# m96-chan/PyGPUkit

Hardware: AMD Instinct MI355X
Metric: decode tokens/sec/GPU + prefill TFLOPS (% MFMA peak), Qwen3-0.6B bf16 (higher is better)
Workload: dtype bf16

## Files before the change

pygpukit_amd/csrc/flash_common.hip.h:

```cpp
#pragma once

#include <type_traits>

#include "attn_plan.h"
#include "pgk_device.hip.h"

namespace pgk {

typedef __bf16 bf16x8_fl __attribute__((ext_vector_type(8)));
typedef _Float16 f16x8_fl __attribute__((ext_vector_type(8)));
typedef float f32x16_fl __attribute__((ext_vector_type(16)));

template <class T> __device__ __forceinline__ f32x16_fl mfma32(const uint4& a, const uint4& b, f32x16_fl c);
template <> __device__ __forceinline__ f32x16_fl mfma32<bf16>(const uint4& a, const uint4& b, f32x16_fl c) {
    return __builtin_amdgcn_mfma_f32_32x32x16_bf16(__builtin_bit_cast(bf16x8_fl, a), __builtin_bit_cast(bf16x8_fl, b), c, 0, 0, 0);
}
template <> __device__ __forceinline__ f32x16_fl mfma32<f16>(const uint4& a, const uint4& b, f32x16_fl c) {
    return __builtin_amdgcn_mfma_f32_32x32x16_f16(__builtin_bit_cast(f16x8_fl, a), __builtin_bit_cast(f16x8_fl, b), c, 0, 0, 0);
}
template <class T> __device__ __forceinline__ uint32_t pack16x2(float lo, float hi);
template <> __device__ __forceinline__ uint32_t pack16x2<bf16>(float lo, float hi) { return pack_bf16x2(lo, hi); }
template <> __device__ __forceinline__ uint32_t pack16x2<f16>(float lo, float hi) {
    return (uint32_t)__builtin_bit_cast(uint16_t, static_cast<_Float16>(lo)) | ((uint32_t)__builtin_bit_cast(uint16_t, static_cast<_Float16>(hi)) << 16);
}

struct FlashPlain {};
struct FlashFull {};
struct FlashIrope {
    const void* positions;
    float attn_scale, floor_scale;
    int causal_offset;
    int pos_is_i64;
};
struct FlashAlibi {
    const float* slopes;
};

__device__ __forceinline__ int fl_v_off(int d, int c8) { return d * 128 + ((c8 ^ ((d >> 1) & 15)) << 3); }

struct FlashSplit {
    int nsplit;
    float* ml;
    void* o;
    uint8_t* q8;
    float* q8s;
};

template <class T, int D>
__global__ __launch_bounds__(256) void flash_merge_kernel(const float* ml, const T* po, T* out, int hq, int q_len, int nsplit, long long oh, long long os,
                                                          uint8_t* q8 = nullptr, float* q8s = nullptr) {
    constexpr int CPR = D / 8;
    const size_t gid = (size_t)blockIdx.x * 256 + threadIdx.x;
    const size_t nrow = (size_t)q_len * hq;
    if (gid >= nrow * CPR) return;
    const size_t rowi = gid / CPR;
    const int c = (int)(gid % CPR), qrow = (int)(rowi / hq), head = (int)(rowi % hq);
    float mstar = -INFINITY;
    for (int s2 = 0; s2 < nsplit; ++s2) mstar = fmaxf(mstar, ml[(((size_t)s2 * hq + head) * q_len + qrow) * 2]);
    float acc[8] = {0.f, 0.f, 0.f, 0.f, 0.f, 0.f, 0.f, 0.f}, den = 0.f;
    for (int s2 = 0; s2 < nsplit; ++s2) {
        const float* r = ml + (((size_t)s2 * hq + head) * q_len + qrow) * 2;
        const float w = (r[1] > 0.f) ? r[1] * __builtin_amdgcn_exp2f(r[0] - mstar) : 0.f;
        if (w > 0.f) {
            Vec<T> v;
            v.load(po + (((size_t)s2 * q_len + qrow) * hq + head) * D + c * 8);
            float f[8];
            v.to_float(f);
#pragma unroll
            for (int j = 0; j < 8; ++j) acc[j] = fmaf(w, f[j], acc[j]);
            den += w;
        }
    }
    const float inv = den > 0.f ? 1.f / den : 0.f;
#pragma unroll
    for (int j = 0; j < 8; ++j) acc[j] *= inv;
    Vec<T> v;
    v.from_float(acc);
    if constexpr (std::is_same<T, bf16>::value && D == 128) {
        if (q8 != nullptr) {
            v.to_float(acc);
            float amax = 0.f;
#pragma unroll
            for (int j = 0; j < 8; ++j) amax = fmaxf(amax, fabsf(acc[j]));
            amax = group16_max(amax);
            const float sc = amax > 0.f ? amax / 448.0f : 1.0f;
            uint2 o8;
            o8.x = pack_fp8x4(acc[0] / sc, acc[1] / sc, acc[2] / sc, acc[3] / sc);
            o8.y = pack_fp8x4(acc[4] / sc, acc[5] / sc, acc[6] / sc, acc[7] / sc);
            *reinterpret_cast<uint2*>(q8 + rowi * D + c * 8) = o8;
            if (c == 0) q8s[rowi] = sc;
            return;
        }
    }
    v.store(out + (size_t)head * oh + (size_t)qrow * os + c * 8);
}

template <class T, int D>
__global__ __launch_bounds__(256) void transpose_v_kernel(const T* v, T* vt, int kv_len, int kv_pad, long long kh, long long ks) {
    __shared__ uint16_t tile[64][D + 2];
    const int kv0 = blockIdx.x * 64, head = blockIdx.y;
    const T* vh = v + (size_t)head * kh;
    constexpr int NC = D / 8;
    for (int c = threadIdx.x; c < 64 * NC; c += 256) {
        const int r = c / NC, kc = c % NC;
        uint4 x = make_uint4(0, 0, 0, 0);
        if (kv0 + r < kv_len) x = *reinterpret_cast<const uint4*>(vh + (size_t)(kv0 + r) * ks + kc * 8);
        const uint32_t w[4] = {x.x, x.y, x.z, x.w};
#pragma unroll
        for (int j = 0; j < 4; ++j) {
            tile[r][kc * 8 + 2 * j] = (uint16_t)(w[j] & 0xFFFFu);
            tile[r][kc * 8 + 2 * j + 1] = (uint16_t)(w[j] >> 16);
        }
    }
    __syncthreads();
    T* oh = vt + (size_t)head * D * kv_pad;
    for (int c = threadIdx.x; c < D * 8; c += 256) {
        const int d = c >> 3, kc = c & 7;
        uint32_t w[4];
#pragma unroll
        for (int j = 0; j < 4; ++j) w[j] = (uint32_t)tile[kc * 8 + 2 * j][d] | ((uint32_t)tile[kc * 8 + 2 * j + 1][d] << 16);
        *reinterpret_cast<uint4*>(oh + (size_t)d * kv_pad + kv0 + kc * 8) = make_uint4(w[0], w[1], w[2], w[3]);
    }
}

}
```

pygpukit_amd/csrc/ops_flash.hip:

```cpp

#include "flash_common.hip.h"

namespace pgk {

template <int D> __device__ __forceinline__ int fl_k_off(int r, int c) { return r * (2 * D) + ((c ^ (r & (D / 8 - 1))) << 4); }

template <class T, int D, class X = FlashPlain>
__global__ __launch_bounds__(FL_THREADS, 2) void flash_fwd_kernel(const T* q, const T* k, const T* vt, T* out, int hq, int hkv,
                                                              int q_len, int kv_len, int kv_pad, float scale_log2e, FlashStrides sd,
                                                              FlashSplit sp, X ex) {
    constexpr bool IROPE = std::is_same<X, FlashIrope>::value;
    constexpr bool ALIBI = std::is_same<X, FlashAlibi>::value;
    constexpr bool FULL = std::is_same<X, FlashFull>::value;
    constexpr int NC = D / 8;
    constexpr int KS = D / 16;
    constexpr int DT = D / 32;
    constexpr int KCH = 64 * NC / FL_THREADS;
    constexpr int VCH = D * 8 / FL_THREADS;
    constexpr int K_BYTES = 64 * D * 2, V_BYTES = D * 128;
    extern __shared__ __attribute__((aligned(16))) char fl_smem[];
    auto Ks = [&](int buf) -> char* { return fl_smem + buf * K_BYTES; };
    auto Vs = [&](int buf) -> char* { return fl_smem + 2 * K_BYTES + buf * V_BYTES; };

    const int tid = threadIdx.x, lane = tid & 63, wid = tid >> 6, ql = lane & 31, h = lane >> 5;
    const int rep = hq / hkv, nqt = (q_len + FL_BQ - 1) / FL_BQ;
    const int id = blockIdx.x;
    const int kvh = id % hkv, rest = id / hkv;
    const int head = kvh * rep + rest % rep;
    const int rest2 = rest / rep;
    int order = rest2;
    const int nord = nqt * sp.nsplit;
    if (sp.nsplit > 1 && order >= nord / 2) order = nord / 2 + (nord - 1 - order);
    const int split = order % sp.nsplit;
    const int qt = nqt - 1 - order / sp.nsplit;
    const int qw0 = qt * FL_BQ + wid * 32;
    int mask_off = kv_len - q_len;
    if constexpr (IROPE) mask_off = ex.causal_offset;
    if constexpr (FULL) mask_off = kv_len;
    const int causal_off = mask_off;
    const T* qh = q + (size_t)head * sd.qh;
    const T* kh = k + (size_t)kvh * sd.kh;
    const T* vh = vt + (size_t)kvh * D * kv_pad;

    uint4 qf[KS];
    {
        const T* qrow = qh + (size_t)min(qw0 + ql, q_len - 1) * sd.qs + 8 * h;
        float qmul = scale_log2e;
        if constexpr (IROPE)
            qmul *= irope_temperature(irope_position(ex.positions, min(qw0 + ql, q_len - 1), ex.pos_is_i64), ex.attn_scale, ex.floor_scale);
#pragma unroll
        for (int ks = 0; ks < KS; ++ks) {
            Vec<T> v;
            v.load(qrow + ks * 16);
            float f[8];
            v.to_float(f);
#pragma unroll
            for (int j = 0; j < 8; ++j) f[j] *= qmul;
            v.from_float(f);
            qf[ks] = v.raw;
        }
    }
    f32x16_fl o[DT];
#pragma unroll
    for (int i = 0; i < DT; ++i)
#pragma unroll
        for (int r = 0; r < 16; ++r) o[i][r] = 0.f;
    float m_run = -INFINITY, l_run = 0.f;
    float slope2 = 0.f;
    if constexpr (ALIBI) slope2 = ex.slopes[head] * 1.4426950408889634f;

    const int q_last = min(qt * FL_BQ + FL_BQ - 1, q_len - 1);
    const int kv_end = min(kv_len, causal_off + q_last + 1);
    const int nt_all = (kv_end + FL_BKV - 1) / FL_BKV;
    const int t0 = (int)((long long)nt_all * split / sp.nsplit), t1 = (int)((long long)nt_all * (split + 1) / sp.nsplit);

    static_assert(KCH == VCH && (KCH == 2 || KCH == 4), "staging is written for D = 64 / 128");
    uint4 rk0, rk1, rk2, rk3, rv0, rv1, rv2, rv3;
    const int kr = tid / NC, kc16 = tid % NC;
    constexpr int KR_STEP = FL_THREADS / NC;
    const int vd = tid >> 3, vc = tid & 7;
    auto k_src = [&](int kv0, int i) { return kh + (size_t)min(kv0 + kr + KR_STEP * i, kv_len - 1) * sd.ks + kc16 * 8; };
    const uint32_t ko0 = (uint32_t)(kr * sd.ks + kc16 * 8), ko_step = (uint32_t)(KR_STEP * sd.ks);
    const uint32_t vo0 = (uint32_t)(vd * kv_pad + vc * 8), vo_step = (uint32_t)(32 * kv_pad);
    auto load_k = [&](int t) {
        const int kv0 = t * FL_BKV;
        if (kv0 + FL_BKV <= kv_len) {
            const T* kt = kh + (size_t)kv0 * sd.ks;
            rk0 = *reinterpret_cast<const uint4*>(kt + ko0);
            rk1 = *reinterpret_cast<const uint4*>(kt + ko0 + ko_step);
            if constexpr (KCH == 4) {
                rk2 = *reinterpret_cast<const uint4*>(kt + ko0 + 2 * ko_step);
                rk3 = *reinterpret_cast<const uint4*>(kt + ko0 + 3 * ko_step);
            }
        } else {
            rk0 = *reinterpret_cast<const uint4*>(k_src(kv0, 0));
            rk1 = *reinterpret_cast<const uint4*>(k_src(kv0, 1));
            if constexpr (KCH == 4) {
                rk2 = *reinterpret_cast<const uint4*>(k_src(kv0, 2));
                rk3 = *reinterpret_cast<const uint4*>(k_src(kv0, 3));
            }
        }
    };
    auto load_v = [&](int t) {
        const T* vtile = vh + t * FL_BKV;
        rv0 = *reinterpret_cast<const uint4*>(vtile + vo0);
        rv1 = *reinterpret_cast<const uint4*>(vtile + vo0 + vo_step);
        if constexpr (VCH == 4) {
            rv2 = *reinterpret_cast<const uint4*>(vtile + vo0 + 2 * vo_step);
            rv3 = *reinterpret_cast<const uint4*>(vtile + vo0 + 3 * vo_step);
        }
    };
    auto put_v = [&](char* base, int d, const uint4& x) {
        *reinterpret_cast<uint2*>(base + fl_v_off(d, 2 * vc)) = make_uint2(x.x, x.y);
        *reinterpret_cast<uint2*>(base + fl_v_off(d, 2 * vc + 1)) = make_uint2(x.z, x.w);
    };
    auto store_k = [&](int buf) {
        char* kb = Ks(buf);
        *reinterpret_cast<uint4*>(kb + fl_k_off<D>(kr, kc16)) = rk0;
        *reinterpret_cast<uint4*>(kb + fl_k_off<D>(kr + KR_STEP, kc16)) = rk1;
        if constexpr (KCH == 4) {
            *reinterpret_cast<uint4*>(kb + fl_k_off<D>(kr + 2 * KR_STEP, kc16)) = rk2;
            *reinterpret_cast<uint4*>(kb + fl_k_off<D>(kr + 3 * KR_STEP, kc16)) = rk3;
        }
    };
    auto store_v = [&](int buf) {
        char* vb = Vs(buf);
        put_v(vb, vd, rv0);
        put_v(vb, vd + 32, rv1);
        if constexpr (VCH == 4) {
            put_v(vb, vd + 64, rv2);
            put_v(vb, vd + 96, rv3);
        }
    };
    auto qk = [&](int buf, int kv0, f32x16_fl& s0, f32x16_fl& s1) {
        if constexpr (ALIBI) {
            const float base = slope2 * (float)(kv0 + 4 * h - (causal_off + qw0 + ql));
#pragma unroll
            for (int r = 0; r < 16; ++r) {
                s0[r] = fmaf(slope2, (float)((r & 3) + 8 * (r >> 2)), base);
                s1[r] = fmaf(slope2, (float)(32 + (r & 3) + 8 * (r >> 2)), base);
            }
        } else {
#pragma unroll
            for (int r = 0; r < 16; ++r) { s0[r] = 0.f; s1[r] = 0.f; }
        }
#pragma unroll
        for (int ks = 0; ks < KS; ++ks) {
            const uint4 a0 = *reinterpret_cast<const uint4*>(Ks(buf) + fl_k_off<D>(ql, 2 * ks + h));
            const uint4 a1 = *reinterpret_cast<const uint4*>(Ks(buf) + fl_k_off<D>(32 + ql, 2 * ks + h));
            s0 = mfma32<T>(a0, qf[ks], s0);
            s1 = mfma32<T>(a1, qf[ks], s1);
        }
    };
    auto live = [&](int t) -> bool { return t < t1 && t * FL_BKV <= causal_off + qw0 + 31; };

    f32x16_fl sc0, sc1;
    if (t0 < t1) {
        load_k(t0);
        load_v(t0);
        store_k(t0 & 1);
        store_v(t0 & 1);
    }
#pragma unroll
    for (int ks = 0; ks < KS; ++ks) asm volatile("" ::"v"(qf[ks].x), "v"(qf[ks].y), "v"(qf[ks].z), "v"(qf[ks].w));
    __syncthreads();
    typedef uint32_t fl_u32x2 __attribute__((ext_vector_type(2)));
    typedef __attribute__((address_space(3))) const volatile fl_u32x2* fl_lds_cv64;
    for (int t = t0; t < t1; ++t) {
        const int buf = t & 1, kv0 = t * FL_BKV;
        if (t + 1 < t1) { load_k(t + 1); load_v(t + 1); }
        const bool cur = live(t);
        if (cur) qk(buf, kv0, sc0, sc1);
        if (cur) {
            const bool need_mask = kv0 + FL_BKV - 1 > causal_off + qw0 || kv0 + FL_BKV > kv_len;
            const int lim = min(causal_off + qw0 + ql, kv_len - 1) - kv0 - 4 * h;
            float mx = -INFINITY;
            if (need_mask) {
#pragma unroll
                for (int r = 0; r < 16; ++r) {
                    const int kvl = (r & 3) + 8 * (r >> 2);
                    sc0[r] = kvl <= lim ? sc0[r] : -INFINITY;
                    sc1[r] = 32 + kvl <= lim ? sc1[r] : -INFINITY;
                }
            }
#pragma unroll
            for (int r = 0; r < 16; r += 2) mx = fmaxf(fmaxf(fmaxf(sc0[r], sc1[r]), fmaxf(sc0[r + 1], sc1[r + 1])), mx);
            mx = fmaxf(mx, __shfl_xor(mx, 32, 64));
            const float m_new = (mx > m_run + 6.0f || m_run == -INFINITY) ? fmaxf(m_run, mx) : m_run;
            const float m_use = m_new == -INFINITY ? 0.f : m_new;
            const bool moved = __builtin_amdgcn_ballot_w64(m_new != m_run) != 0;
            const float alpha = moved ? __builtin_amdgcn_exp2f(m_run - m_use) : 1.0f;
            float ls = 0.f;
#pragma unroll
            for (int r = 0; r < 16; ++r) {
                sc0[r] = __builtin_amdgcn_exp2f(sc0[r] - m_use);
                sc1[r] = __builtin_amdgcn_exp2f(sc1[r] - m_use);
                ls += sc0[r] + sc1[r];
            }
            l_run = l_run * alpha + ls;
            m_run = m_new;
            if (moved) {
#pragma unroll
                for (int i = 0; i < DT; ++i)
#pragma unroll
                    for (int r = 0; r < 16; ++r) o[i][r] *= alpha;
            }
            const char* vrow = Vs(buf) + ql * 128;
            const int vsw = (ql >> 1) & 15;
#pragma unroll
            for (int s = 0; s < 4; ++s) {
                uint4 pb;
                if (s < 2) {
                    pb = make_uint4(pack16x2<T>(sc0[8 * s + 0], sc0[8 * s + 1]), pack16x2<T>(sc0[8 * s + 2], sc0[8 * s + 3]),
                                    pack16x2<T>(sc0[8 * s + 4], sc0[8 * s + 5]), pack16x2<T>(sc0[8 * s + 6], sc0[8 * s + 7]));
                } else {
                    pb = make_uint4(pack16x2<T>(sc1[8 * (s - 2) + 0], sc1[8 * (s - 2) + 1]), pack16x2<T>(sc1[8 * (s - 2) + 2], sc1[8 * (s - 2) + 3]),
                                    pack16x2<T>(sc1[8 * (s - 2) + 4], sc1[8 * (s - 2) + 5]), pack16x2<T>(sc1[8 * (s - 2) + 6], sc1[8 * (s - 2) + 7]));
                }
#pragma unroll
                for (int i = 0; i < DT; ++i) {
                    const fl_u32x2 lo = *(fl_lds_cv64)(vrow + (((4 * s + h) ^ vsw) << 3) + i * 4096);
                    const fl_u32x2 hi = *(fl_lds_cv64)(vrow + (((4 * s + 2 + h) ^ vsw) << 3) + i * 4096);
                    o[i] = mfma32<T>(make_uint4(lo.x, lo.y, hi.x, hi.y), pb, o[i]);
                }
            }
        }
        if (t + 1 < t1) { store_k(buf ^ 1); store_v(buf ^ 1); }
        __syncthreads();
    }

    const float l_tot = l_run + __shfl_xor(l_run, 32, 64);
    const float inv = l_tot > 0.f ? 1.f / l_tot : 0.f;
    const int qrow = qw0 + ql;
    if constexpr (std::is_same<T, bf16>::value && D == 128 && std::is_same<X, FlashPlain>::value) {
        if (sp.q8 != nullptr && sp.nsplit == 1) {
            float amax = 0.f;
#pragma unroll
            for (int i = 0; i < DT; ++i)
#pragma unroll
                for (int e = 0; e < 16; ++e) {
                    o[i][e] = __uint_as_float(pack_bf16x2(o[i][e] * inv, 0.f) << 16);
                    amax = fmaxf(amax, fabsf(o[i][e]));
                }
            amax = fmaxf(amax, __shfl_xor(amax, 32, 64));
            const float sc = amax > 0.f ? amax / 448.0f : 1.0f;
            if (qrow < q_len) {
                uint8_t* qrow8 = sp.q8 + ((size_t)qrow * hq + head) * D;
#pragma unroll
                for (int i = 0; i < DT; ++i)
#pragma unroll
                    for (int g = 0; g < 4; ++g)
                        *reinterpret_cast<uint32_t*>(qrow8 + i * 32 + 8 * g + 4 * h) =
                            pack_fp8x4(o[i][4 * g] / sc, o[i][4 * g + 1] / sc, o[i][4 * g + 2] / sc, o[i][4 * g + 3] / sc);
                if (h == 0) sp.q8s[(size_t)qrow * hq + head] = sc;
            }
            return;
        }
    }
    if (qrow < q_len) {
        T* orow = sp.nsplit > 1 ? reinterpret_cast<T*>(sp.o) + (((size_t)split * q_len + qrow) * hq + head) * D
                                : out + (size_t)head * sd.oh + (size_t)qrow * sd.os;
#pragma unroll
        for (int i = 0; i < DT; ++i)
#pragma unroll
            for (int g = 0; g < 4; ++g) {
                uint2 w;
                w.x = pack16x2<T>(o[i][4 * g] * inv, o[i][4 * g + 1] * inv);
                w.y = pack16x2<T>(o[i][4 * g + 2] * inv, o[i][4 * g + 3] * inv);
                *reinterpret_cast<uint2*>(orow + i * 32 + 8 * g + 4 * h) = w;
            }
        if (sp.nsplit > 1 && h == 0) {
            float* ml = sp.ml + (((size_t)split * hq + head) * q_len + qrow) * 2;
            ml[0] = m_run;
            ml[1] = l_tot;
        }
    }
}

template <class T, int D, class X = FlashPlain>
static pgk_status flash_launch(const T* q, const T* k, const T* v, T* out, int hq, int hkv, int q_len, int kv_len, float scale,
                               const FlashStrides& sd, hipStream_t st, uint8_t* q8 = nullptr, float* q8s = nullptr, X ex = X{},
                               int kv_seen = 0) {
    const int kv_pad = ceil_div(kv_len, 64) * 64;
    const int nqt = ceil_div(q_len, FL_BQ);
    const int nsplit = flash_nsplit(nqt, hq, kv_seen > 0 ? kv_seen : kv_len, device_cu_count());
    const size_t vt_bytes = (size_t)hkv * D * kv_pad * sizeof(T);
    const size_t po_bytes = nsplit > 1 ? (size_t)nsplit * q_len * hq * D * sizeof(T) : 0;
    const size_t ml_bytes = nsplit > 1 ? (size_t)nsplit * hq * q_len * 2 * sizeof(float) : 0;
    void* ws = nullptr;
    if (pgk_status r = pgk_malloc(&ws, vt_bytes + po_bytes + ml_bytes + 512)) return r;
    char* base = (char*)ws;
    T* vt = (T*)base;
    FlashSplit sp{nsplit, nullptr, nullptr, q8, q8s};
    if (nsplit > 1) {
        sp.o = base + ((vt_bytes + 255) & ~(size_t)255);
        sp.ml = (float*)((char*)sp.o + ((po_bytes + 255) & ~(size_t)255));
    }
    transpose_v_kernel<T, D><<<dim3(kv_pad / 64, hkv), 256, 0, st>>>(v, vt, kv_len, kv_pad, sd.kh, sd.ks);
    constexpr size_t LDS = 2 * (size_t)(64 * D * 2) + 2 * (size_t)(D * 128);
    static bool attr_done = false;
    if (LDS > 48 * 1024 && !attr_done) {
        PGK_CHECK_HIP(hipFuncSetAttribute(reinterpret_cast<const void*>(&flash_fwd_kernel<T, D, X>),
                                          hipFuncAttributeMaxDynamicSharedMemorySize, (int)LDS));
        attr_done = true;
    }
    flash_fwd_kernel<T, D, X><<<nqt * hq * nsplit, FL_THREADS, LDS, st>>>(q, k, (const T*)vt, out, hq, hkv, q_len, kv_len, kv_pad,
                                                                         scale * 1.4426950408889634f, sd, sp, ex);
    hipError_t e = hipGetLastError();
    if (e == hipSuccess && nsplit > 1) {
        const size_t work = (size_t)q_len * hq * (D / 8);
        flash_merge_kernel<T, D><<<(unsigned)((work + 255) / 256), 256, 0, st>>>(sp.ml, (const T*)sp.o, out, hq, q_len, nsplit, sd.oh, sd.os, q8, q8s);
        e = hipGetLastError();
    }
    pgk_free(ws);
    PGK_CHECK_HIP(e);
    return PGK_OK;
}

template <class X>
static pgk_status flash_launch_any(int dt16, int d, const void* q, const void* k, const void* v, void* out, int hq, int hkv, int q_len,
                                   int kv_len, float scale, const FlashStrides& sd, hipStream_t st, X ex, int kv_seen) {
    auto run = [&](auto* t, auto dd) {
        using T = std::remove_pointer_t<decltype(t)>;
        return flash_launch<T, decltype(dd)::value, X>((const T*)q, (const T*)k, (const T*)v, (T*)out, hq, hkv, q_len, kv_len, scale, sd, st,
                                                       nullptr, nullptr, ex, kv_seen);
    };
    const std::integral_constant<int, 128> d128;
    const std::integral_constant<int, 64> d64;
    if (dt16 == 0) return d == 128 ? run((bf16*)nullptr, d128) : run((bf16*)nullptr, d64);
    return d == 128 ? run((f16*)nullptr, d128) : run((f16*)nullptr, d64);
}

pgk_status flash_prefill(const void* q, const void* k, const void* v, void* out, int hq, int hkv, int q_len, int kv_len, int d, float scale,
                         const FlashStrides& sd, int dt16, hipStream_t st) {
    return flash_launch_any(dt16, d, q, k, v, out, hq, hkv, q_len, kv_len, scale, sd, st, FlashPlain{}, 0);
}

pgk_status flash_prefill_full(const void* q, const void* k, const void* v, void* out, int hq, int hkv, int q_len, int kv_len, int d,
                              float scale, const FlashStrides& sd, int dt16, hipStream_t st) {
    return flash_launch_any(dt16, d, q, k, v, out, hq, hkv, q_len, kv_len, scale, sd, st, FlashFull{}, kv_len);
}

pgk_status flash_prefill_irope(const void* q, const void* k, const void* v, const void* positions, void* out, int hq, int hkv, int q_len,
                               int kv_len, int d, float attn_scale, float floor_scale, int causal_offset, const FlashStrides& sd,
                               int pos_is_i64, int dt16, hipStream_t st) {
    const int off = causal_offset < kv_len ? causal_offset : kv_len;
    const FlashIrope ex{positions, attn_scale, floor_scale, off, pos_is_i64};
// ... 18 lines not shown
```

pygpukit_amd/csrc/ops_flash_fp8.hip:

```cpp

#include "flash_common.hip.h"

namespace pgk {

typedef int i32x8_f8 __attribute__((ext_vector_type(8)));

struct Fp8HeadSrc {
    const bf16* x;
    uint8_t* codes;
    uint8_t* scale_bytes;
    uint32_t* amax;
    int heads, rows;
    long long sh, ss;
};

__device__ __forceinline__ int fp8_head_exp(uint32_t a) {
    if (a == 0) return 0;
    const int e = (int)(a >> 7) - 135 + ((a & 127u) > 96u ? 1 : 0);
    return max(-127, min(127, e));
}

__global__ __launch_bounds__(256) void fp8_head_absmax_kernel(Fp8HeadSrc a, Fp8HeadSrc b) {
    const bool second = (int)blockIdx.y >= a.heads;
    const Fp8HeadSrc t = second ? b : a;
// ... 19 lines not shown
    const int e = fp8_head_exp(t.amax[head]);
    if (blockIdx.x == 0 && threadIdx.x == 0) t.scale_bytes[head] = (uint8_t)(e + 127);
    const float mul = __uint_as_float(e < 127 ? (uint32_t)(127 - e) << 23 : 0x00400000u);
    const bf16* xh = t.x + (size_t)head * t.sh;
    uint8_t* ch = t.codes + (size_t)head * t.rows * 128;
    const long long nchunk = (long long)t.rows * 16;
    for (long long c = (long long)blockIdx.x * 256 + threadIdx.x; c < nchunk; c += (long long)gridDim.x * 256) {
        Vec<bf16> v;
        v.load(xh + (c >> 4) * t.ss + (c & 15) * 8);
        float f[8];
        v.to_float(f);
#pragma unroll
        for (int j = 0; j < 8; ++j) f[j] = fminf(fmaxf(f[j] * mul, -448.0f), 448.0f);
        *reinterpret_cast<uint2*>(ch + c * 8) = make_uint2(pack_fp8x4(f[0], f[1], f[2], f[3]), pack_fp8x4(f[4], f[5], f[6], f[7]));
    }
}

static pgk_status fp8_quantize_heads(const Fp8HeadSrc& a, const Fp8HeadSrc& b, hipStream_t st) {
    const long long chunks = 16LL * (a.rows > b.rows || b.heads == 0 ? a.rows : b.rows);
    const int blocks = (int)min(64LL, (chunks + 1023) / 1024);
    const dim3 grid(blocks, a.heads + b.heads);
    fp8_head_absmax_kernel<<<grid, 256, 0, st>>>(a, b);
    fp8_head_codes_kernel<<<grid, 256, 0, st>>>(a, b);
    PGK_LAUNCH_CHECK();
    return PGK_OK;
}

__device__ __forceinline__ int fl8_k_off(int r, int c) { return r * 128 + ((c ^ ((r >> 1) & 7)) << 4); }

constexpr int FL8_K_BYTES = 64 * 128, FL8_V_BYTES = 128 * 128;
constexpr size_t FL8_LDS = 2 * (size_t)FL8_K_BYTES + 2 * (size_t)FL8_V_BYTES;

__global__ __launch_bounds__(FL_THREADS, 2) void flash_fwd_fp8_kernel(const uint8_t* q8, const uint8_t* k8, const uint8_t* qsb, const uint8_t* ksb,
                                                                  const bf16* vt, bf16* out, int hq, int hkv, int q_len, int kv_len,
                                                                  int kv_pad, float scale_log2e, FlashStrides sd, FlashSplit sp) {
    typedef bf16 T;
    constexpr int D = 128, DT = D / 32;
    extern __shared__ __attribute__((aligned(16))) char fl8_smem[];
    auto Ks = [&](int buf) -> char* { return fl8_smem + buf * FL8_K_BYTES; };
    auto Vs = [&](int buf) -> char* { return fl8_smem + 2 * FL8_K_BYTES + buf * FL8_V_BYTES; };

    const int tid = threadIdx.x, lane = tid & 63, wid = tid >> 6, ql = lane & 31, h = lane >> 5;
    const int rep = hq / hkv, nqt = (q_len + FL_BQ - 1) / FL_BQ;
    const int id = blockIdx.x;
    const int kvh = id % hkv, rest = id / hkv;
    const int head = kvh * rep + rest % rep;
    const int rest2 = rest / rep;
    int order = rest2;
    const int nord = nqt * sp.nsplit;
    if (sp.nsplit > 1 && order >= nord / 2) order = nord / 2 + (nord - 1 - order);
    const int split = order % sp.nsplit;
    const int qt = nqt - 1 - order / sp.nsplit;
    const int qw0 = qt * FL_BQ + wid * 32;
    const int causal_off = kv_len - q_len;
    const uint8_t* kh = k8 + (size_t)kvh * kv_len * D;
    const T* vh = vt + (size_t)kvh * D * kv_pad;
    const float cf = fminf(fmaxf(ldexpf(scale_log2e, (int)qsb[head] + (int)ksb[kvh] - 254), 1.17549435e-38f), 3.40282347e+38f);

    i32x8_f8 qf0, qf1;
    {
        const uint8_t* qrow = q8 + ((size_t)head * q_len + min(qw0 + ql, q_len - 1)) * D + 32 * h;
        const uint4 a0 = *reinterpret_cast<const uint4*>(qrow), a1 = *reinterpret_cast<const uint4*>(qrow + 16);
        const uint4 b0 = *reinterpret_cast<const uint4*>(qrow + 64), b1 = *reinterpret_cast<const uint4*>(qrow + 80);
        qf0 = i32x8_f8{(int)a0.x, (int)a0.y, (int)a0.z, (int)a0.w, (int)a1.x, (int)a1.y, (int)a1.z, (int)a1.w};
        qf1 = i32x8_f8{(int)b0.x, (int)b0.y, (int)b0.z, (int)b0.w, (int)b1.x, (int)b1.y, (int)b1.z, (int)b1.w};
    }
    f32x16_fl o[DT];
#pragma unroll
    for (int i = 0; i < DT; ++i)
#pragma unroll
        for (int r = 0; r < 16; ++r) o[i][r] = 0.f;
    float m_run = -INFINITY, l_run = 0.f;

    const int q_last = min(qt * FL_BQ + FL_BQ - 1, q_len - 1);
    const int kv_end = min(kv_len, causal_off + q_last + 1);
    const int nt_all = (kv_end + FL_BKV - 1) / FL_BKV;
    const int t0 = (int)((long long)nt_all * split / sp.nsplit), t1 = (int)((long long)nt_all * (split + 1) / sp.nsplit);

    uint4 rk0, rk1, rv0, rv1, rv2, rv3;
    const int kr = tid >> 3, kc = tid & 7;
    const int vd = tid >> 3, vc = tid & 7;
    const uint32_t vo0 = (uint32_t)(vd * kv_pad + vc * 8), vo_step = (uint32_t)(32 * kv_pad);
    auto load_k = [&](int t) {
        const int kv0 = t * FL_BKV;
        if (kv0 + FL_BKV <= kv_len) {
            const uint8_t* kt = kh + (size_t)kv0 * D + tid * 16;
            rk0 = *reinterpret_cast<const uint4*>(kt);
            rk1 = *reinterpret_cast<const uint4*>(kt + 4096);
        } else {
            rk0 = *reinterpret_cast<const uint4*>(kh + (size_t)min(kv0 + kr, kv_len - 1) * D + kc * 16);
            rk1 = *reinterpret_cast<const uint4*>(kh + (size_t)min(kv0 + kr + 32, kv_len - 1) * D + kc * 16);
        }
    };
    auto load_v = [&](int t) {
        const T* vtile = vh + t * FL_BKV;
        rv0 = *reinterpret_cast<const uint4*>(vtile + vo0);
        rv1 = *reinterpret_cast<const uint4*>(vtile + vo0 + vo_step);
        rv2 = *reinterpret_cast<const uint4*>(vtile + vo0 + 2 * vo_step);
        rv3 = *reinterpret_cast<const uint4*>(vtile + vo0 + 3 * vo_step);
    };
    auto put_v = [&](char* base, int d, const uint4& x) {
        *reinterpret_cast<uint2*>(base + fl_v_off(d, 2 * vc)) = make_uint2(x.x, x.y);
        *reinterpret_cast<uint2*>(base + fl_v_off(d, 2 * vc + 1)) = make_uint2(x.z, x.w);
    };
    auto store_k = [&](int buf) {
        char* kb = Ks(buf);
        *reinterpret_cast<uint4*>(kb + fl8_k_off(kr, kc)) = rk0;
        *reinterpret_cast<uint4*>(kb + fl8_k_off(kr + 32, kc)) = rk1;
    };
    auto store_v = [&](int buf) {
        char* vb = Vs(buf);
        put_v(vb, vd, rv0);
        put_v(vb, vd + 32, rv1);
        put_v(vb, vd + 64, rv2);
        put_v(vb, vd + 96, rv3);
    };
    auto k_frag = [&](int buf, int row, int s) -> i32x8_f8 {
        const uint4 lo = *reinterpret_cast<const uint4*>(Ks(buf) + fl8_k_off(row, 4 * s + 2 * h));
        const uint4 hi = *reinterpret_cast<const uint4*>(Ks(buf) + fl8_k_off(row, 4 * s + 2 * h + 1));
        return i32x8_f8{(int)lo.x, (int)lo.y, (int)lo.z, (int)lo.w, (int)hi.x, (int)hi.y, (int)hi.z, (int)hi.w};
    };
    auto qk = [&](int buf, f32x16_fl& s0, f32x16_fl& s1) {
#pragma unroll
        for (int r = 0; r < 16; ++r) { s0[r] = 0.f; s1[r] = 0.f; }
        const i32x8_f8 a00 = k_frag(buf, ql, 0), a10 = k_frag(buf, 32 + ql, 0);
        const i32x8_f8 a01 = k_frag(buf, ql, 1), a11 = k_frag(buf, 32 + ql, 1);
        s0 = __builtin_amdgcn_mfma_scale_f32_32x32x64_f8f6f4(a00, qf0, s0, 0, 0, 0, 0, 0, 0);
        s1 = __builtin_amdgcn_mfma_scale_f32_32x32x64_f8f6f4(a10, qf0, s1, 0, 0, 0, 0, 0, 0);
        s0 = __builtin_amdgcn_mfma_scale_f32_32x32x64_f8f6f4(a01, qf1, s0, 0, 0, 0, 0, 0, 0);
        s1 = __builtin_amdgcn_mfma_scale_f32_32x32x64_f8f6f4(a11, qf1, s1, 0, 0, 0, 0, 0, 0);
    };
    auto live = [&](int t) -> bool { return t < t1 && t * FL_BKV <= causal_off + qw0 + 31; };

    f32x16_fl sc0, sc1;
    if (t0 < t1) {
        load_k(t0);
        load_v(t0);
        store_k(t0 & 1);
        store_v(t0 & 1);
    }
#pragma unroll
    for (int j = 0; j < 8; ++j) asm volatile("" ::"v"(qf0[j]), "v"(qf1[j]));
    __syncthreads();
    typedef uint32_t fl_u32x2 __attribute__((ext_vector_type(2)));
    typedef __attribute__((address_space(3))) const volatile fl_u32x2* fl_lds_cv64;
    for (int t = t0; t < t1; ++t) {
        const int buf = t & 1, kv0 = t * FL_BKV;
        if (t + 1 < t1) { load_k(t + 1); load_v(t + 1); }
        const bool cur = live(t);
        if (cur) qk(buf, sc0, sc1);
        if (cur) {
            const bool need_mask = kv0 + FL_BKV - 1 > causal_off + qw0 || kv0 + FL_BKV > kv_len;
            const int lim = min(causal_off + qw0 + ql, kv_len - 1) - kv0 - 4 * h;
            float mx = -INFINITY;
            if (need_mask) {
#pragma unroll
                for (int r = 0; r < 16; ++r) {
                    const int kvl = (r & 3) + 8 * (r >> 2);
                    sc0[r] = kvl <= lim ? sc0[r] : -INFINITY;
                    sc1[r] = 32 + kvl <= lim ? sc1[r] : -INFINITY;
                }
            }
#pragma unroll
            for (int r = 0; r < 16; r += 2) mx = fmaxf(fmaxf(fmaxf(sc0[r], sc1[r]), fmaxf(sc0[r + 1], sc1[r + 1])), mx);
            mx = fmaxf(mx, __shfl_xor(mx, 32, 64)) * cf;
            const float m_new = (mx > m_run + 6.0f || m_run == -INFINITY) ? fmaxf(m_run, mx) : m_run;
            const float m_use = m_new == -INFINITY ? 0.f : m_new;
            const bool moved = __builtin_amdgcn_ballot_w64(m_new != m_run) != 0;
            const float alpha = moved ? __builtin_amdgcn_exp2f(m_run - m_use) : 1.0f;
            float ls = 0.f;
#pragma unroll
            for (int r = 0; r < 16; ++r) {
                sc0[r] = __builtin_amdgcn_exp2f(__builtin_fmaf(sc0[r], cf, -m_use));
                sc1[r] = __builtin_amdgcn_exp2f(__builtin_fmaf(sc1[r], cf, -m_use));
                ls += sc0[r] + sc1[r];
            }
            l_run = l_run * alpha + ls;
            m_run = m_new;
            if (moved) {
#pragma unroll
                for (int i = 0; i < DT; ++i)
#pragma unroll
                    for (int r = 0; r < 16; ++r) o[i][r] *= alpha;
            }
            const char* vrow = Vs(buf) + ql * 128;
            const int vsw = (ql >> 1) & 15;
#pragma unroll
            for (int s = 0; s < 4; ++s) {
                uint4 pb;
                if (s < 2) {
                    pb = make_uint4(pack_bf16x2(sc0[8 * s + 0], sc0[8 * s + 1]), pack_bf16x2(sc0[8 * s + 2], sc0[8 * s + 3]),
                                    pack_bf16x2(sc0[8 * s + 4], sc0[8 * s + 5]), pack_bf16x2(sc0[8 * s + 6], sc0[8 * s + 7]));
                } else {
                    pb = make_uint4(pack_bf16x2(sc1[8 * (s - 2) + 0], sc1[8 * (s - 2) + 1]), pack_bf16x2(sc1[8 * (s - 2) + 2], sc1[8 * (s - 2) + 3]),
                                    pack_bf16x2(sc1[8 * (s - 2) + 4], sc1[8 * (s - 2) + 5]), pack_bf16x2(sc1[8 * (s - 2) + 6], sc1[8 * (s - 2) + 7]));
                }
#pragma unroll
                for (int i = 0; i < DT; ++i) {
                    const fl_u32x2 lo = *(fl_lds_cv64)(vrow + (((4 * s + h) ^ vsw) << 3) + i * 4096);
                    const fl_u32x2 hi = *(fl_lds_cv64)(vrow + (((4 * s + 2 + h) ^ vsw) << 3) + i * 4096);
                    o[i] = mfma32<T>(make_uint4(lo.x, lo.y, hi.x, hi.y), pb, o[i]);
                }
            }
        }
        if (t + 1 < t1) { store_k(buf ^ 1); store_v(buf ^ 1); }
        __syncthreads();
    }

    const float l_tot = l_run + __shfl_xor(l_run, 32, 64);
    const float inv = l_tot > 0.f ? 1.f / l_tot : 0.f;
    const int qrow = qw0 + ql;
    if (qrow < q_len) {
        T* orow = sp.nsplit > 1 ? reinterpret_cast<T*>(sp.o) + (((size_t)split * q_len + qrow) * hq + head) * D
                                : out + (size_t)head * sd.oh + (size_t)qrow * sd.os;
#pragma unroll
        for (int i = 0; i < DT; ++i)
#pragma unroll
            for (int g = 0; g < 4; ++g) {
                uint2 w;
                w.x = pack_bf16x2(o[i][4 * g] * inv, o[i][4 * g + 1] * inv);
                w.y = pack_bf16x2(o[i][4 * g + 2] * inv, o[i][4 * g + 3] * inv);
                *reinterpret_cast<uint2*>(orow + i * 32 + 8 * g + 4 * h) = w;
            }
        if (sp.nsplit > 1 && h == 0) {
            float* ml = sp.ml + (((size_t)split * hq + head) * q_len + qrow) * 2;
            ml[0] = m_run;
            ml[1] = l_tot;
        }
    }
}

static size_t up256(size_t n) { return (n + 255) & ~(size_t)255; }

static pgk_status flash_fp8_launch(const bf16* q, const bf16* k, const bf16* v, bf16* out, int hq, int hkv, int q_len, int kv_len, float scale,
                                   const FlashStrides& sd, hipStream_t st) {
    constexpr int D = 128;
    const int kv_pad = ceil_div(kv_len, 64) * 64;
    const int nqt = ceil_div(q_len, FL_BQ);
    const int nsplit = flash_nsplit(nqt, hq, kv_len, device_cu_count());
    const size_t vt_bytes = up256((size_t)hkv * D * kv_pad * sizeof(bf16));
    const size_t po_bytes = nsplit > 1 ? up256((size_t)nsplit * q_len * hq * D * sizeof(bf16)) : 0;
    const size_t ml_bytes = nsplit > 1 ? up256((size_t)nsplit * hq * q_len * 2 * sizeof(float)) : 0;
    const size_t q8_bytes = up256((size_t)hq * q_len * D), k8_bytes = up256((size_t)hkv * kv_len * D);
    const size_t am_bytes = up256((size_t)(hq + hkv) * sizeof(uint32_t)), sb_bytes = up256((size_t)(hq + hkv));
    void* ws = nullptr;
    if (pgk_status r = pgk_malloc(&ws, vt_bytes + po_bytes + ml_bytes + q8_bytes + k8_bytes + am_bytes + sb_bytes)) return r;
    char* p = (char*)ws;
    bf16* vt = (bf16*)p; p += vt_bytes;
    FlashSplit sp{nsplit, nullptr, nullptr, nullptr, nullptr};
    if (nsplit > 1) {
        sp.o = p; p += po_bytes;
        sp.ml = (float*)p; p += ml_bytes;
    }
    uint8_t* q8 = (uint8_t*)p; p += q8_bytes;
    uint8_t* k8 = (uint8_t*)p; p += k8_bytes;
    uint32_t* amax = (uint32_t*)p; p += am_bytes;
    uint8_t* sb = (uint8_t*)p;
    hipError_t e = hipMemsetAsync(amax, 0, (size_t)(hq + hkv) * sizeof(uint32_t), st);
    pgk_status r = PGK_OK;
    if (e == hipSuccess) {
        const Fp8HeadSrc qs{q, q8, sb, amax, hq, q_len, sd.qh, sd.qs}, ks{k, k8, sb + hq, amax + hq, hkv, kv_len, sd.kh, sd.ks};
        r = fp8_quantize_heads(qs, ks, st);
    }
    if (e == hipSuccess && r == PGK_OK) {
        transpose_v_kernel<bf16, D><<<dim3(kv_pad / 64, hkv), 256, 0, st>>>(v, vt, kv_len, kv_pad, sd.kh, sd.ks);
        flash_fwd_fp8_kernel<<<nqt * hq * nsplit, FL_THREADS, FL8_LDS, st>>>(q8, k8, sb, sb + hq, vt, out, hq, hkv, q_len, kv_len, kv_pad,
                                                                            scale * 1.4426950408889634f, sd, sp);
        e = hipGetLastError();
        if (e == hipSuccess && nsplit > 1) {
            const size_t work = (size_t)q_len * hq * (D / 8);
            flash_merge_kernel<bf16, D><<<(unsigned)((work + 255) / 256), 256, 0, st>>>(sp.ml, (const bf16*)sp.o, out, hq, q_len, nsplit, sd.oh, sd.os);
            e = hipGetLastError();
        }
    }
    pgk_free(ws);
    if (r != PGK_OK) return r;
    PGK_CHECK_HIP(e);
    return PGK_OK;
}

}

extern "C" {

pgk_status pgk_sdpa_causal_fp8(const void* q, const void* k, const void* v, void* out, int hq, int hkv, int q_len, int kv_len, int d,
                               float scale, int64_t q_stride_h, int64_t q_stride_s, int64_t kv_stride_h, int64_t kv_stride_s,
                               int64_t o_stride_h, int64_t o_stride_s, pgk_dtype dt, pgk_stream s) {
    using namespace pgk;
    PGK_REQUIRE(q && k && v && out, "pgk_sdpa_causal_fp8: null pointer");
    PGK_REQUIRE(dt == PGK_BF16, "pgk_sdpa_causal_fp8: bfloat16 only (dtype %d)", (int)dt);
    PGK_REQUIRE(d == 128, "pgk_sdpa_causal_fp8: head_dim must be 128 (got %d)", d);
    PGK_REQUIRE(hq > 0 && hkv > 0 && hq % hkv == 0, "pgk_sdpa_causal_fp8: n_heads mismatch (Hq=%d, Hkv=%d)", hq, hkv);
    PGK_REQUIRE(q_len > 0 && kv_len > 0, "pgk_sdpa_causal_fp8: bad shape q_len=%d kv_len=%d", q_len, kv_len);
    PGK_REQUIRE(kv_len >= q_len, "pgk_sdpa_causal_fp8: kv_len %d < q_len %d", kv_len, q_len);
    PGK_REQUIRE(aligned16(q) && aligned16(k) && aligned16(v) && aligned16(out) &&
                    ((q_stride_h | q_stride_s | kv_stride_h | kv_stride_s | o_stride_h | o_stride_s) & 7) == 0,
                "pgk_sdpa_causal_fp8: pointers must be 16-byte aligned and strides multiples of 8 elements");
    if (scale <= 0.f) scale = 1.0f / sqrtf((float)d);
    const FlashStrides sd{q_stride_h, q_stride_s, kv_stride_h, kv_stride_s, o_stride_h, o_stride_s};
// ... 30 lines not shown
```

Before: 1701.

## Drop V transpose kernel; read row-major V via LDS transpose loads

Removes the separate transpose_v pre-pass and its workspace allocation. The flash kernels now load V row-major, in the same pattern as K, into a swizzled LDS image and use ds_read_tr16_b64 to produce the transposed MFMA B-fragments. This saves a kernel launch, a full global read and write of V, and in the non-split case a workspace malloc. The cost is new swizzle and fragment-offset logic that must match the hardware transpose-read semantics.

```diff
diff --git a/pygpukit_amd/csrc/flash_common.hip.h b/pygpukit_amd/csrc/flash_common.hip.h
--- a/pygpukit_amd/csrc/flash_common.hip.h
+++ b/pygpukit_amd/csrc/flash_common.hip.h
@@ -36,7 +36,18 @@
     const float* slopes;
 };
 
-__device__ __forceinline__ int fl_v_off(int d, int c8) { return d * 128 + ((c8 ^ ((d >> 1) & 15)) << 3); }
+template <int D> __device__ __forceinline__ int fl_v_off(int r, int c) {
+    static_assert(D == 64 || D == 128, "V image: 128- or 256-byte rows");
+    return r * (2 * D) + ((c ^ ((D == 128 ? (r & 3) : ((r >> 1) & 1)) << 2)) << 4);
+}
+template <int D> __device__ __forceinline__ int fl_v_frag_off(int lane, int i) {
+    const int q = (lane >> 2) & 3, p = lane & 3, g1 = (lane >> 4) & 1, h = lane >> 5;
+    return fl_v_off<D>(4 * h + q, 4 * i + 2 * g1 + (p >> 1)) + 8 * (p & 1);
+}
+typedef short fl_v4s __attribute__((ext_vector_type(4)));
+__device__ __forceinline__ uint2 fl_v_read_tr(const char* lds_addr) {
+    return __builtin_bit_cast(uint2, __builtin_amdgcn_ds_read_tr16_b64_v4i16((__attribute__((address_space(3))) fl_v4s*)lds_addr));
+}
 
 struct FlashSplit {
     int nsplit;
@@ -95,32 +106,4 @@
     v.store(out + (size_t)head * oh + (size_t)qrow * os + c * 8);
 }
 
-template <class T, int D>
-__global__ __launch_bounds__(256) void transpose_v_kernel(const T* v, T* vt, int kv_len, int kv_pad, long long kh, long long ks) {
-    __shared__ uint16_t tile[64][D + 2];
-    const int kv0 = blockIdx.x * 64, head = blockIdx.y;
-    const T* vh = v + (size_t)head * kh;
-    constexpr int NC = D / 8;
-    for (int c = threadIdx.x; c < 64 * NC; c += 256) {
-        const int r = c / NC, kc = c % NC;
-        uint4 x = make_uint4(0, 0, 0, 0);
-        if (kv0 + r < kv_len) x = *reinterpret_cast<const uint4*>(vh + (size_t)(kv0 + r) * ks + kc * 8);
-        const uint32_t w[4] = {x.x, x.y, x.z, x.w};
-#pragma unroll
-        for (int j = 0; j < 4; ++j) {
-            tile[r][kc * 8 + 2 * j] = (uint16_t)(w[j] & 0xFFFFu);
-            tile[r][kc * 8 + 2 * j + 1] = (uint16_t)(w[j] >> 16);
-        }
-    }
-    __syncthreads();
-    T* oh = vt + (size_t)head * D * kv_pad;
-    for (int c = threadIdx.x; c < D * 8; c += 256) {
-        const int d = c >> 3, kc = c & 7;
-        uint32_t w[4];
-#pragma unroll
-        for (int j = 0; j < 4; ++j) w[j] = (uint32_t)tile[kc * 8 + 2 * j][d] | ((uint32_t)tile[kc * 8 + 2 * j + 1][d] << 16);
-        *reinterpret_cast<uint4*>(oh + (size_t)d * kv_pad + kv0 + kc * 8) = make_uint4(w[0], w[1], w[2], w[3]);
-    }
 }
-
-}
diff --git a/pygpukit_amd/csrc/ops_flash.hip b/pygpukit_amd/csrc/ops_flash.hip
--- a/pygpukit_amd/csrc/ops_flash.hip
+++ b/pygpukit_amd/csrc/ops_flash.hip
@@ -6,8 +6,8 @@
 template <int D> __device__ __forceinline__ int fl_k_off(int r, int c) { return r * (2 * D) + ((c ^ (r & (D / 8 - 1))) << 4); }
 
 template <class T, int D, class X = FlashPlain>
-__global__ __launch_bounds__(FL_THREADS, 2) void flash_fwd_kernel(const T* q, const T* k, const T* vt, T* out, int hq, int hkv,
-                                                              int q_len, int kv_len, int kv_pad, float scale_log2e, FlashStrides sd,
+__global__ __launch_bounds__(FL_THREADS, 2) void flash_fwd_kernel(const T* q, const T* k, const T* v, T* out, int hq, int hkv,
+                                                              int q_len, int kv_len, float scale_log2e, FlashStrides sd,
                                                               FlashSplit sp, X ex) {
     constexpr bool IROPE = std::is_same<X, FlashIrope>::value;
     constexpr bool ALIBI = std::is_same<X, FlashAlibi>::value;
@@ -16,8 +16,8 @@
     constexpr int KS = D / 16;
     constexpr int DT = D / 32;
     constexpr int KCH = 64 * NC / FL_THREADS;
-    constexpr int VCH = D * 8 / FL_THREADS;
-    constexpr int K_BYTES = 64 * D * 2, V_BYTES = D * 128;
+    constexpr int VCH = KCH;
+    constexpr int K_BYTES = 64 * D * 2, V_BYTES = 64 * D * 2;
     extern __shared__ __attribute__((aligned(16))) char fl_smem[];
     auto Ks = [&](int buf) -> char* { return fl_smem + buf * K_BYTES; };
     auto Vs = [&](int buf) -> char* { return fl_smem + 2 * K_BYTES + buf * V_BYTES; };
@@ -40,7 +40,7 @@
     const int causal_off = mask_off;
     const T* qh = q + (size_t)head * sd.qh;
     const T* kh = k + (size_t)kvh * sd.kh;
-    const T* vh = vt + (size_t)kvh * D * kv_pad;
+    const T* vh = v + (size_t)kvh * sd.kh;
 
     uint4 qf[KS];
     {
@@ -78,10 +78,8 @@
     uint4 rk0, rk1, rk2, rk3, rv0, rv1, rv2, rv3;
     const int kr = tid / NC, kc16 = tid % NC;
     constexpr int KR_STEP = FL_THREADS / NC;
-    const int vd = tid >> 3, vc = tid & 7;
-    auto k_src = [&](int kv0, int i) { return kh + (size_t)min(kv0 + kr + KR_STEP * i, kv_len - 1) * sd.ks + kc16 * 8; };
+    auto kv_src = [&](const T* base, int kv0, int i) { return base + (size_t)min(kv0 + kr + KR_STEP * i, kv_len - 1) * sd.ks + kc16 * 8; };
     const uint32_t ko0 = (uint32_t)(kr * sd.ks + kc16 * 8), ko_step = (uint32_t)(KR_STEP * sd.ks);
-    const uint32_t vo0 = (uint32_t)(vd * kv_pad + vc * 8), vo_step = (uint32_t)(32 * kv_pad);
     auto load_k = [&](int t) {
         const int kv0 = t * FL_BKV;
         if (kv0 + FL_BKV <= kv_len) {
@@ -93,26 +91,32 @@
                 rk3 = *reinterpret_cast<const uint4*>(kt + ko0 + 3 * ko_step);
             }
         } else {
-            rk0 = *reinterpret_cast<const uint4*>(k_src(kv0, 0));
-            rk1 = *reinterpret_cast<const uint4*>(k_src(kv0, 1));
+            rk0 = *reinterpret_cast<const uint4*>(kv_src(kh, kv0, 0));
+            rk1 = *reinterpret_cast<const uint4*>(kv_src(kh, kv0, 1));
             if constexpr (KCH == 4) {
-                rk2 = *reinterpret_cast<const uint4*>(k_src(kv0, 2));
-                rk3 = *reinterpret_cast<const uint4*>(k_src(kv0, 3));
+                rk2 = *reinterpret_cast<const uint4*>(kv_src(kh, kv0, 2));
+                rk3 = *reinterpret_cast<const uint4*>(kv_src(kh, kv0, 3));
             }
         }
     };
     auto load_v = [&](int t) {
-        const T* vtile = vh + t * FL_BKV;
-        rv0 = *reinterpret_cast<const uint4*>(vtile + vo0);
-        rv1 = *reinterpret_cast<const uint4*>(vtile + vo0 + vo_step);
-        if constexpr (VCH == 4) {
-            rv2 = *reinterpret_cast<const uint4*>(vtile + vo0 + 2 * vo_step);
-            rv3 = *reinterpret_cast<const uint4*>(vtile + vo0 + 3 * vo_step);
-        }
-    };
-    auto put_v = [&](char* base, int d, const uint4& x) {
-        *reinterpret_cast<uint2*>(base + fl_v_off(d, 2 * vc)) = make_uint2(x.x, x.y);
-        *reinterpret_cast<uint2*>(base + fl_v_off(d, 2 * vc + 1)) = make_uint2(x.z, x.w);
+        const int kv0 = t * FL_BKV;
+        if (kv0 + FL_BKV <= kv_len) {
+            const T* vtile = vh + (size_t)kv0 * sd.ks;
+            rv0 = *reinterpret_cast<const uint4*>(vtile + ko0);
+            rv1 = *reinterpret_cast<const uint4*>(vtile + ko0 + ko_step);
+            if constexpr (VCH == 4) {
+                rv2 = *reinterpret_cast<const uint4*>(vtile + ko0 + 2 * ko_step);
+                rv3 = *reinterpret_cast<const uint4*>(vtile + ko0 + 3 * ko_step);
+            }
+        } else {
+            rv0 = *reinterpret_cast<const uint4*>(kv_src(vh, kv0, 0));
+            rv1 = *reinterpret_cast<const uint4*>(kv_src(vh, kv0, 1));
+            if constexpr (VCH == 4) {
+                rv2 = *reinterpret_cast<const uint4*>(kv_src(vh, kv0, 2));
+                rv3 = *reinterpret_cast<const uint4*>(kv_src(vh, kv0, 3));
+            }
+        }
     };
     auto store_k = [&](int buf) {
         char* kb = Ks(buf);
@@ -125,11 +129,11 @@
     };
     auto store_v = [&](int buf) {
         char* vb = Vs(buf);
-        put_v(vb, vd, rv0);
-        put_v(vb, vd + 32, rv1);
+        *reinterpret_cast<uint4*>(vb + fl_v_off<D>(kr, kc16)) = rv0;
+        *reinterpret_cast<uint4*>(vb + fl_v_off<D>(kr + KR_STEP, kc16)) = rv1;
         if constexpr (VCH == 4) {
-            put_v(vb, vd + 64, rv2);
-            put_v(vb, vd + 96, rv3);
+            *reinterpret_cast<uint4*>(vb + fl_v_off<D>(kr + 2 * KR_STEP, kc16)) = rv2;
+            *reinterpret_cast<uint4*>(vb + fl_v_off<D>(kr + 3 * KR_STEP, kc16)) = rv3;
         }
     };
     auto qk = [&](int buf, int kv0, f32x16_fl& s0, f32x16_fl& s1) {
@@ -164,8 +168,9 @@
 #pragma unroll
     for (int ks = 0; ks < KS; ++ks) asm volatile("" ::"v"(qf[ks].x), "v"(qf[ks].y), "v"(qf[ks].z), "v"(qf[ks].w));
     __syncthreads();
-    typedef uint32_t fl_u32x2 __attribute__((ext_vector_type(2)));
-    typedef __attribute__((address_space(3))) const volatile fl_u32x2* fl_lds_cv64;
+    int vfo[DT];
+#pragma unroll
+    for (int i = 0; i < DT; ++i) vfo[i] = fl_v_frag_off<D>(lane, i);
     for (int t = t0; t < t1; ++t) {
         const int buf = t & 1, kv0 = t * FL_BKV;
         if (t + 1 < t1) { load_k(t + 1); load_v(t + 1); }
@@ -205,8 +210,7 @@
 #pragma unroll
                     for (int r = 0; r < 16; ++r) o[i][r] *= alpha;
             }
-            const char* vrow = Vs(buf) + ql * 128;
-            const int vsw = (ql >> 1) & 15;
+            const char* vb = Vs(buf);
 #pragma unroll
             for (int s = 0; s < 4; ++s) {
                 uint4 pb;
@@ -219,8 +223,8 @@
                 }
 #pragma unroll
                 for (int i = 0; i < DT; ++i) {
-                    const fl_u32x2 lo = *(fl_lds_cv64)(vrow + (((4 * s + h) ^ vsw) << 3) + i * 4096);
-                    const fl_u32x2 hi = *(fl_lds_cv64)(vrow + (((4 * s + 2 + h) ^ vsw) << 3) + i * 4096);
+                    const uint2 lo = fl_v_read_tr(vb + vfo[i] + (16 * s) * (2 * D));
+                    const uint2 hi = fl_v_read_tr(vb + vfo[i] + (16 * s + 8) * (2 * D));
                     o[i] = mfma32<T>(make_uint4(lo.x, lo.y, hi.x, hi.y), pb, o[i]);
                 }
             }
@@ -281,30 +285,25 @@
 static pgk_status flash_launch(const T* q, const T* k, const T* v, T* out, int hq, int hkv, int q_len, int kv_len, float scale,
                                const FlashStrides& sd, hipStream_t st, uint8_t* q8 = nullptr, float* q8s = nullptr, X ex = X{},
                                int kv_seen = 0) {
-    const int kv_pad = ceil_div(kv_len, 64) * 64;
     const int nqt = ceil_div(q_len, FL_BQ);
     const int nsplit = flash_nsplit(nqt, hq, kv_seen > 0 ? kv_seen : kv_len, device_cu_count());
-    const size_t vt_bytes = (size_t)hkv * D * kv_pad * sizeof(T);
     const size_t po_bytes = nsplit > 1 ? (size_t)nsplit * q_len * hq * D * sizeof(T) : 0;
     const size_t ml_bytes = nsplit > 1 ? (size_t)nsplit * hq * q_len * 2 * sizeof(float) : 0;
-    void* ws = nullptr;
-    if (pgk_status r = pgk_malloc(&ws, vt_bytes + po_bytes + ml_bytes + 512)) return r;
-    char* base = (char*)ws;
-    T* vt = (T*)base;
-    FlashSplit sp{nsplit, nullptr, nullptr, q8, q8s};
-    if (nsplit > 1) {
-        sp.o = base + ((vt_bytes + 255) & ~(size_t)255);
-        sp.ml = (float*)((char*)sp.o + ((po_bytes + 255) & ~(size_t)255));
-    }
-    transpose_v_kernel<T, D><<<dim3(kv_pad / 64, hkv), 256, 0, st>>>(v, vt, kv_len, kv_pad, sd.kh, sd.ks);
-    constexpr size_t LDS = 2 * (size_t)(64 * D * 2) + 2 * (size_t)(D * 128);
+    constexpr size_t LDS = 4 * (size_t)(64 * D * 2);
     static bool attr_done = false;
     if (LDS > 48 * 1024 && !attr_done) {
         PGK_CHECK_HIP(hipFuncSetAttribute(reinterpret_cast<const void*>(&flash_fwd_kernel<T, D, X>),
                                           hipFuncAttributeMaxDynamicSharedMemorySize, (int)LDS));
         attr_done = true;
     }
-    flash_fwd_kernel<T, D, X><<<nqt * hq * nsplit, FL_THREADS, LDS, st>>>(q, k, (const T*)vt, out, hq, hkv, q_len, kv_len, kv_pad,
+    void* ws = nullptr;
+    FlashSplit sp{nsplit, nullptr, nullptr, q8, q8s};
+    if (nsplit > 1) {
+        if (pgk_status r = pgk_malloc(&ws, po_bytes + ml_bytes + 512)) return r;
+        sp.o = ws;
+        sp.ml = (float*)((char*)ws + ((po_bytes + 255) & ~(size_t)255));
+    }
+    flash_fwd_kernel<T, D, X><<<nqt * hq * nsplit, FL_THREADS, LDS, st>>>(q, k, v, out, hq, hkv, q_len, kv_len,
                                                                          scale * 1.4426950408889634f, sd, sp, ex);
     hipError_t e = hipGetLastError();
     if (e == hipSuccess && nsplit > 1) {
@@ -312,7 +311,7 @@
         flash_merge_kernel<T, D><<<(unsigned)((work + 255) / 256), 256, 0, st>>>(sp.ml, (const T*)sp.o, out, hq, q_len, nsplit, sd.oh, sd.os, q8, q8s);
         e = hipGetLastError();
     }
-    pgk_free(ws);
+    if (ws) pgk_free(ws);
     PGK_CHECK_HIP(e);
     return PGK_OK;
 }
diff --git a/pygpukit_amd/csrc/ops_flash_fp8.hip b/pygpukit_amd/csrc/ops_flash_fp8.hip
--- a/pygpukit_amd/csrc/ops_flash_fp8.hip
+++ b/pygpukit_amd/csrc/ops_flash_fp8.hip
@@ -75,8 +75,8 @@
 constexpr size_t FL8_LDS = 2 * (size_t)FL8_K_BYTES + 2 * (size_t)FL8_V_BYTES;
 
 __global__ __launch_bounds__(FL_THREADS, 2) void flash_fwd_fp8_kernel(const uint8_t* q8, const uint8_t* k8, const uint8_t* qsb, const uint8_t* ksb,
-                                                                  const bf16* vt, bf16* out, int hq, int hkv, int q_len, int kv_len,
-                                                                  int kv_pad, float scale_log2e, FlashStrides sd, FlashSplit sp) {
+                                                                  const bf16* v, bf16* out, int hq, int hkv, int q_len, int kv_len,
+                                                                  float scale_log2e, FlashStrides sd, FlashSplit sp) {
     typedef bf16 T;
     constexpr int D = 128, DT = D / 32;
     extern __shared__ __attribute__((aligned(16))) char fl8_smem[];
@@ -97,7 +97,7 @@
     const int qw0 = qt * FL_BQ + wid * 32;
     const int causal_off = kv_len - q_len;
     const uint8_t* kh = k8 + (size_t)kvh * kv_len * D;
-    const T* vh = vt + (size_t)kvh * D * kv_pad;
+    const T* vh = v + (size_t)kvh * sd.kh;
     const float cf = fminf(fmaxf(ldexpf(scale_log2e, (int)qsb[head] + (int)ksb[kvh] - 254), 1.17549435e-38f), 3.40282347e+38f);
 
     i32x8_f8 qf0, qf1;
@@ -122,8 +122,9 @@
 
     uint4 rk0, rk1, rv0, rv1, rv2, rv3;
     const int kr = tid >> 3, kc = tid & 7;
-    const int vd = tid >> 3, vc = tid & 7;
-    const uint32_t vo0 = (uint32_t)(vd * kv_pad + vc * 8), vo_step = (uint32_t)(32 * kv_pad);
+    const int vr = tid >> 4, vc = tid & 15;
+    const uint32_t vo0 = (uint32_t)(vr * sd.ks + vc * 8), vo_step = (uint32_t)(16 * sd.ks);
+    auto v_src = [&](int kv0, int i) { return vh + (size_t)min(kv0 + vr + 16 * i, kv_len - 1) * sd.ks + vc * 8; };
     auto load_k = [&](int t) {
         const int kv0 = t * FL_BKV;
         if (kv0 + FL_BKV <= kv_len) {
@@ -136,15 +137,19 @@
         }
     };
     auto load_v = [&](int t) {
-        const T* vtile = vh + t * FL_BKV;
-        rv0 = *reinterpret_cast<const uint4*>(vtile + vo0);
-        rv1 = *reinterpret_cast<const uint4*>(vtile + vo0 + vo_step);
-        rv2 = *reinterpret_cast<const uint4*>(vtile + vo0 + 2 * vo_step);
-        rv3 = *reinterpret_cast<const uint4*>(vtile + vo0 + 3 * vo_step);
-    };
-    auto put_v = [&](char* base, int d, const uint4& x) {
-        *reinterpret_cast<uint2*>(base + fl_v_off(d, 2 * vc)) = make_uint2(x.x, x.y);
-        *reinterpret_cast<uint2*>(base + fl_v_off(d, 2 * vc + 1)) = make_uint2(x.z, x.w);
+        const int kv0 = t * FL_BKV;
+        if (kv0 + FL_BKV <= kv_len) {
+            const T* vtile = vh + (size_t)kv0 * sd.ks;
+            rv0 = *reinterpret_cast<const uint4*>(vtile + vo0);
+            rv1 = *reinterpret_cast<const uint4*>(vtile + vo0 + vo_step);
+            rv2 = *reinterpret_cast<const uint4*>(vtile + vo0 + 2 * vo_step);
+            rv3 = *reinterpret_cast<const uint4*>(vtile + vo0 + 3 * vo_step);
+        } else {
+            rv0 = *reinterpret_cast<const uint4*>(v_src(kv0, 0));
+            rv1 = *reinterpret_cast<const uint4*>(v_src(kv0, 1));
+            rv2 = *reinterpret_cast<const uint4*>(v_src(kv0, 2));
+            rv3 = *reinterpret_cast<const uint4*>(v_src(kv0, 3));
+        }
     };
     auto store_k = [&](int buf) {
         char* kb = Ks(buf);
@@ -153,10 +158,10 @@
     };
     auto store_v = [&](int buf) {
         char* vb = Vs(buf);
-        put_v(vb, vd, rv0);
-        put_v(vb, vd + 32, rv1);
-        put_v(vb, vd + 64, rv2);
-        put_v(vb, vd + 96, rv3);
+        *reinterpret_cast<uint4*>(vb + fl_v_off<D>(vr, vc)) = rv0;
+        *reinterpret_cast<uint4*>(vb + fl_v_off<D>(vr + 16, vc)) = rv1;
+        *reinterpret_cast<uint4*>(vb + fl_v_off<D>(vr + 32, vc)) = rv2;
+        *reinterpret_cast<uint4*>(vb + fl_v_off<D>(vr + 48, vc)) = rv3;
     };
     auto k_frag = [&](int buf, int row, int s) -> i32x8_f8 {
         const uint4 lo = *reinterpret_cast<const uint4*>(Ks(buf) + fl8_k_off(row, 4 * s + 2 * h));
@@ -185,8 +190,9 @@
 #pragma unroll
     for (int j = 0; j < 8; ++j) asm volatile("" ::"v"(qf0[j]), "v"(qf1[j]));
     __syncthreads();
-    typedef uint32_t fl_u32x2 __attribute__((ext_vector_type(2)));
-    typedef __attribute__((address_space(3))) const volatile fl_u32x2* fl_lds_cv64;
+    int vfo[DT];
+#pragma unroll
+    for (int i = 0; i < DT; ++i) vfo[i] = fl_v_frag_off<D>(lane, i);
     for (int t = t0; t < t1; ++t) {
         const int buf = t & 1, kv0 = t * FL_BKV;
         if (t + 1 < t1) { load_k(t + 1); load_v(t + 1); }
@@ -226,8 +232,7 @@
 #pragma unroll
                     for (int r = 0; r < 16; ++r) o[i][r] *= alpha;
             }
-            const char* vrow = Vs(buf) + ql * 128;
-            const int vsw = (ql >> 1) & 15;
+            const char* vb = Vs(buf);
 #pragma unroll
             for (int s = 0; s < 4; ++s) {
                 uint4 pb;
@@ -240,8 +245,8 @@
                 }
 #pragma unroll
                 for (int i = 0; i < DT; ++i) {
-                    const fl_u32x2 lo = *(fl_lds_cv64)(vrow + (((4 * s + h) ^ vsw) << 3) + i * 4096);
-                    const fl_u32x2 hi = *(fl_lds_cv64)(vrow + (((4 * s + 2 + h) ^ vsw) << 3) + i * 4096);
+                    const uint2 lo = fl_v_read_tr(vb + vfo[i] + (16 * s) * (2 * D));
+                    const uint2 hi = fl_v_read_tr(vb + vfo[i] + (16 * s + 8) * (2 * D));
                     o[i] = mfma32<T>(make_uint4(lo.x, lo.y, hi.x, hi.y), pb, o[i]);
                 }
             }
@@ -278,18 +283,15 @@
 static pgk_status flash_fp8_launch(const bf16* q, const bf16* k, const bf16* v, bf16* out, int hq, int hkv, int q_len, int kv_len, float scale,
                                    const FlashStrides& sd, hipStream_t st) {
     constexpr int D = 128;
-    const int kv_pad = ceil_div(kv_len, 64) * 64;
     const int nqt = ceil_div(q_len, FL_BQ);
     const int nsplit = flash_nsplit(nqt, hq, kv_len, device_cu_count());
-    const size_t vt_bytes = up256((size_t)hkv * D * kv_pad * sizeof(bf16));
     const size_t po_bytes = nsplit > 1 ? up256((size_t)nsplit * q_len * hq * D * sizeof(bf16)) : 0;
     const size_t ml_bytes = nsplit > 1 ? up256((size_t)nsplit * hq * q_len * 2 * sizeof(float)) : 0;
     const size_t q8_bytes = up256((size_t)hq * q_len * D), k8_bytes = up256((size_t)hkv * kv_len * D);
     const size_t am_bytes = up256((size_t)(hq + hkv) * sizeof(uint32_t)), sb_bytes = up256((size_t)(hq + hkv));
     void* ws = nullptr;
-    if (pgk_status r = pgk_malloc(&ws, vt_bytes + po_bytes + ml_bytes + q8_bytes + k8_bytes + am_bytes + sb_bytes)) return r;
+    if (pgk_status r = pgk_malloc(&ws, po_bytes + ml_bytes + q8_bytes + k8_bytes + am_bytes + sb_bytes)) return r;
     char* p = (char*)ws;
-    bf16* vt = (bf16*)p; p += vt_bytes;
     FlashSplit sp{nsplit, nullptr, nullptr, nullptr, nullptr};
     if (nsplit > 1) {
         sp.o = p; p += po_bytes;
@@ -306,8 +308,7 @@
         r = fp8_quantize_heads(qs, ks, st);
     }
     if (e == hipSuccess && r == PGK_OK) {
-        transpose_v_kernel<bf16, D><<<dim3(kv_pad / 64, hkv), 256, 0, st>>>(v, vt, kv_len, kv_pad, sd.kh, sd.ks);
-        flash_fwd_fp8_kernel<<<nqt * hq * nsplit, FL_THREADS, FL8_LDS, st>>>(q8, k8, sb, sb + hq, vt, out, hq, hkv, q_len, kv_len, kv_pad,
+        flash_fwd_fp8_kernel<<<nqt * hq * nsplit, FL_THREADS, FL8_LDS, st>>>(q8, k8, sb, sb + hq, v, out, hq, hkv, q_len, kv_len,
                                                                             scale * 1.4426950408889634f, sd, sp);
         e = hipGetLastError();
         if (e == hipSuccess && nsplit > 1) {
```

Result: no change. 1701, median of 3 (+0.0%).
